# vwxyzjn/cleanrl

Measured on NVIDIA H100. Metric: env steps/sec (SPS) PPO Breakout num_envs=1024, higher is better.
Workload: dtype bf16

## Files before the change

### cleanrl_b200/csrc/net_tc.cu

```cuda
#include <cuda.h>
#include <algorithm>
#include "tc_base.cuh"
#include "tc_conv_win.cuh"
#include "tc_conv23.cuh"
#include "tc_conv1_u8.cuh"
#include "tc_gemm_tma.cuh"
#include "tc_wgrad_win.cuh"
#include "tc_reduce.cuh"
#include "tc_aux.cuh"
#include "tc_heads.cuh"
#include "tc_heads_wide.cuh"
#include "tc_lstm.cuh"

namespace b200rl {

struct NatureLayout {
    int A;
    int64_t c1w, c1b, c2w, c2b, c3w, c3b, fcw, fcb, hw, hb, total;
    int64_t w1f, w2f, w2dg, w3f, w3dg, wfcf, wfcdg, w1l, w1sc, packed_total;
    bool wide; int G; int64_t whf, whdg, hbp;
    int64_t wih, whh, bih, bhh, whhp;
    explicit NatureLayout(int A_) : A(A_), wih(-1), whh(-1), bih(-1), bhh(-1), whhp(-1) {
        int64_t o = 0;
        c1w = o; o += 32 * 4 * 8 * 8;  c1b = o; o += 32;
// ... 406 lines not shown
                   "naturecnn_backward: bad obs_format %d", obs_format);
    B200RL_REQUIRE(obs_format != B200RL_OBS_S2D_U8 || (obs_aux && aligned(obs_aux, 16)), "naturecnn_backward: the uint8 rollout needs obs_aux");
    const NatureLayout L(A);
    const NatureActs Q(n, obs_format == B200RL_OBS_U8_NCHW);
    const bf16* P = reinterpret_cast<const bf16*>(packed);
    bf16* act = reinterpret_cast<bf16*>(acts);
    cudaStream_t s = (cudaStream_t)stream;
    const bf16* x0 = obs_format == B200RL_OBS_U8_NCHW ? act + Q.x0 : reinterpret_cast<const bf16*>(obs);
    const int64_t* x0rows = obs_format == B200RL_OBS_U8_NCHW ? nullptr : rows;
    const size_t big = (naturecnn_big_bytes(n, L) + 255) & ~(size_t)255;
    float* wsbig = reinterpret_cast<float*>(workspace);
    float* wssmall = reinterpret_cast<float*>(reinterpret_cast<char*>(workspace) + big);
    int rc;
    const int A1 = A + 1;
    if (L.wide) {
        ProfScope ps(s, "heads_bwd", 4.0 * n * 512 * A1, (double)n * (2048 + 64 + 8 * A1));
        if ((rc = wide_head_bwd(L, P, dhead, n, A1, act + Q.hid, act + Q.dhid, reinterpret_cast<const uint32_t*>(act + Q.m4),
                                grads + L.hw, grads + L.hb, wsbig, wssmall, s))) return rc;
    } else
    {
        ProfScope ps(s, "heads_bwd", 4.0 * n * 512 * A1, (double)n * (2048 + 64 + 8 * A1));
        if ((rc = heads_bwd_weight<512>(dhead, act + Q.hid, n, A1, wssmall, grads + L.hw, grads + L.hb, s, "naturecnn/heads_bwd"))) return rc;
        if ((rc = heads_bwd_data<512>(dhead, params + L.hw, reinterpret_cast<const uint8_t*>(act + Q.m4), n, A1, act + Q.dhid, s,
                                      "naturecnn/heads_bwd"))) return rc;
    }
    if ((rc = trunk_bwd(L, Q, P, act, grads, n, wsbig, wssmall, tail_ready_event, obs_format == B200RL_OBS_S2D_U8, s))) return rc;
    const bool u8 = obs_format == B200RL_OBS_S2D_U8;
    const WPlan pl = conv1_wgrad_plan(n, u8);
    if (u8) {
        Conv21BwdU8Params cw;
        memset(&cw, 0, sizeof(cw));
        cw.rows = rows; cw.n = (int)n; cw.rows_per_cta = pl.rows_per_cta; cw.ws = wsbig; cw.wsb = wssmall;
        cw.w2dg = P + L.w2dg; cw.m1 = reinterpret_cast<const uint32_t*>(act + Q.m1);
        { ProfScope ps(s, "conv21_bwd", 2.0 * 2.0 * n * 400 * 32 * 256, (double)n * (7744 * 2 + 1600 + 28224 + 14112 * 2));
          if ((rc = launch_conv21_bwd_u8(cw, obs, rows ? (int64_t)1 << 24 : n, act + Q.dact2b, act + Q.dact1, pl.splits, s,
                                         "naturecnn/conv21_bwd_u8"))) return rc; }
    } else {
        WGradWinParams gw;
        wgw_defaults(gw);
        gw.X = x0; gw.rows = x0rows; gw.M = n * 512; gw.n = (int)n; gw.G = 441; gw.cpr = 1; gw.nslots = 4; gw.WRX = round8(128 + 22);
        gw.tpi_shift = 2; gw.n_images = x0rows ? (int64_t)1 << 24 : n;
        gw.shift[0] = 0; gw.shift[1] = 1; gw.shift[2] = 21; gw.shift[3] = 22;
        for (int k = 0; k < 4; ++k) { gw.slot_tap[k] = k; gw.slot_cc[k] = 0; }
        gw.Y = act + Q.dact1; gw.ldy = 32; gw.ncolsY = 32;
        gw.rows_per_cta = pl.rows_per_cta; gw.ws = wsbig; gw.wsb = wssmall;
        { ProfScope ps(s, "conv1_wgrad", 2.0 * n * 400 * 32 * 256, (double)n * (28224 + 14112) * 2);
          if ((rc = launch_wgrad_win(gw, pl.splits, s, "naturecnn/conv1_wgrad"))) return rc; }
    }
    FoldWin fw;
    memset(&fw, 0, sizeof(fw));
    fw.layer = 1; fw.S = pl.splits; fw.nslots = 4; fw.Cout = 32;
    fw.scale = u8 ? 1.0f / 255.0f / kDact1Scale : 1.0f / 255.0f;
    fw.bscale = u8 ? 1.0f / kDact1Scale : 1.f;
    for (int k = 0; k < 4; ++k) fw.slot_tap[k] = k;
    { ProfScope ps(s, "wgrad_fold_bias", 0, 0);
      fw.wsb = wssmall; fw.db = grads + L.c1b;
      tc_fold_win<<<(unsigned)ceil_div(256 * 32 + 32, 32), 256, 0, s>>>(wsbig, fw, grads + L.c1w);
      if ((rc = check_launch("naturecnn/conv1_fold"))) return rc; }
    return B200RL_OK;
}

namespace b200rl {
constexpr int64_t kLstmMaxRows = (int64_t)1 << 17;

struct LstmActs {
    NatureActs T;
    int64_t gx, hseq, hm, save, cm, dgates, total;
    explicit LstmActs(int64_t M) : T(M, false) {
// ... 194 lines not shown
```

### cleanrl_b200/csrc/tc_base.cuh

```cuda
#pragma once
#include <cuda.h>
#include <cstring>
#include "common.cuh"
#include "tc_common.cuh"

namespace b200rl {
using namespace tc;
typedef __nv_bfloat16 bf16;

__device__ __forceinline__ int4 ldg16(const void* p) { return __ldg(reinterpret_cast<const int4*>(p)); }

typedef CUresult (*EncodeTiledFn)(CUtensorMap*, CUtensorMapDataType, cuuint32_t, void*, const cuuint64_t*, const cuuint64_t*,
                                  const cuuint32_t*, const cuuint32_t*, CUtensorMapInterleave, CUtensorMapSwizzle,
                                  CUtensorMapL2promotion, CUtensorMapFloatOOBfill);
static EncodeTiledFn g_encode = nullptr;
static int make_tmap_2d(CUtensorMap* tm, const void* base, int64_t rows, int64_t cols, int box_rows, const char* what) {
    if (!g_encode) {
        void* fn = nullptr;
        cudaDriverEntryPointQueryResult qres;
        cudaError_t e = cudaGetDriverEntryPoint("cuTensorMapEncodeTiled", &fn, cudaEnableDefault, &qres);
        if (e != cudaSuccess || qres != cudaDriverEntryPointSuccess || !fn)
            return fail(B200RL_ERR_CUDA, "%s: cuTensorMapEncodeTiled not available (%s)", what, cudaGetErrorString(e));
        g_encode = reinterpret_cast<EncodeTiledFn>(fn);
    }
    const cuuint64_t dims[2] = {(cuuint64_t)cols, (cuuint64_t)rows};
    const cuuint64_t strides[1] = {(cuuint64_t)cols * 2};
    const cuuint32_t box[2] = {64u, (cuuint32_t)box_rows};
    const cuuint32_t estr[2] = {1u, 1u};
    CUresult r = g_encode(tm, CU_TENSOR_MAP_DATA_TYPE_BFLOAT16, 2, const_cast<void*>(base), dims, strides, box, estr,
                          CU_TENSOR_MAP_INTERLEAVE_NONE, CU_TENSOR_MAP_SWIZZLE_128B, CU_TENSOR_MAP_L2_PROMOTION_L2_256B,
                          CU_TENSOR_MAP_FLOAT_OOB_FILL_NONE);
    if (r != CUDA_SUCCESS) return fail(B200RL_ERR_CUDA, "%s: cuTensorMapEncodeTiled failed (%d)", what, (int)r);
    return B200RL_OK;
}

static int make_tmap_3d(CUtensorMap* tm, const void* base, int64_t n_images, int64_t rows_per_image, int64_t cols, int box_rows,
                        const char* what) {
    if (!g_encode) {
        CUtensorMap dummy;
        int rc = make_tmap_2d(&dummy, base, 128, 64, 8, what);
        if (rc) return rc;
    }
    const cuuint64_t dims[3] = {(cuuint64_t)cols, (cuuint64_t)rows_per_image, (cuuint64_t)n_images};
    const cuuint64_t strides[2] = {(cuuint64_t)cols * 2, (cuuint64_t)rows_per_image * (cuuint64_t)cols * 2};
    const cuuint32_t box[3] = {64u, (cuuint32_t)box_rows, 1u};
    const cuuint32_t estr[3] = {1u, 1u, 1u};
    CUresult r = g_encode(tm, CU_TENSOR_MAP_DATA_TYPE_BFLOAT16, 3, const_cast<void*>(base), dims, strides, box, estr,
                          CU_TENSOR_MAP_INTERLEAVE_NONE, CU_TENSOR_MAP_SWIZZLE_128B, CU_TENSOR_MAP_L2_PROMOTION_L2_256B,
                          CU_TENSOR_MAP_FLOAT_OOB_FILL_NONE);
    if (r != CUDA_SUCCESS) return fail(B200RL_ERR_CUDA, "%s: cuTensorMapEncodeTiled (3-D) failed (%d)", what, (int)r);
    return B200RL_OK;
}

static int make_tmap_3d_u8(CUtensorMap* tm, const void* base, int64_t n_images, int64_t rows_per_image, int64_t cols, int64_t pitch,
                           int box_rows, int box_cols, const char* what) {
    if (!g_encode) {
        CUtensorMap dummy;
        int rc = make_tmap_2d(&dummy, base, 128, 64, 8, what);
        if (rc) return rc;
    }
    const cuuint64_t dims[3] = {(cuuint64_t)cols, (cuuint64_t)rows_per_image, (cuuint64_t)n_images};
    const cuuint64_t strides[2] = {(cuuint64_t)pitch, (cuuint64_t)rows_per_image * (cuuint64_t)pitch};
    const cuuint32_t box[3] = {(cuuint32_t)box_cols, (cuuint32_t)box_rows, 1u};
    const cuuint32_t estr[3] = {1u, 1u, 1u};
    CUresult r = g_encode(tm, CU_TENSOR_MAP_DATA_TYPE_UINT8, 3, const_cast<void*>(base), dims, strides, box, estr,
                          CU_TENSOR_MAP_INTERLEAVE_NONE,
                          box_cols == 64 ? CU_TENSOR_MAP_SWIZZLE_64B : (box_cols == 128 ? CU_TENSOR_MAP_SWIZZLE_128B : CU_TENSOR_MAP_SWIZZLE_NONE),
                          CU_TENSOR_MAP_L2_PROMOTION_L2_256B, CU_TENSOR_MAP_FLOAT_OOB_FILL_NONE);
    if (r != CUDA_SUCCESS) return fail(B200RL_ERR_CUDA, "%s: cuTensorMapEncodeTiled (u8 3-D) failed (%d)", what, (int)r);
    return B200RL_OK;
}

static int make_tmap_pairs_u8(CUtensorMap* tm, const void* base, int64_t n_images, int box_rows, bool swizzle, const char* what) {
    if (!g_encode) {
        CUtensorMap dummy;
        int rc = make_tmap_2d(&dummy, base, 128, 64, 8, what);
        if (rc) return rc;
    }
    const cuuint64_t dims[3] = {128u, 221u, (cuuint64_t)n_images};
    const cuuint64_t strides[2] = {128u, 28224u};
    const cuuint32_t box[3] = {128u, (cuuint32_t)box_rows, 1u};
    const cuuint32_t estr[3] = {1u, 1u, 1u};
    CUresult r = g_encode(tm, CU_TENSOR_MAP_DATA_TYPE_UINT8, 3, const_cast<void*>(base), dims, strides, box, estr,
// ... 33 lines not shown
```

### cleanrl_b200/csrc/tc_common.cuh

```cuda
#pragma once
#include <cuda_bf16.h>
#include <cstdint>
#include "tc_wgmma.cuh"

namespace b200rl { namespace tc {

__device__ __forceinline__ uint32_t smem_u32(const void* p) {
    return static_cast<uint32_t>(__cvta_generic_to_shared(p));
}

__device__ __forceinline__ void mbar_init(uint64_t* bar, uint32_t count) {
    asm volatile("mbarrier.init.shared::cta.b64 [%0], %1;" ::"r"(smem_u32(bar)), "r"(count) : "memory");
}
__device__ __forceinline__ void fence_barrier_init() {
    asm volatile("fence.mbarrier_init.release.cluster;" ::: "memory");
}
__device__ __forceinline__ bool mbar_try_wait(uint64_t* bar, uint32_t parity) {
    uint32_t ok;
    asm volatile(
        "{\n\t.reg .pred p;\n\t"
        "mbarrier.try_wait.parity.shared::cta.b64 p, [%1], %2;\n\t"
        "selp.u32 %0, 1, 0, p;\n\t}\n"
        : "=r"(ok)
        : "r"(smem_u32(bar)), "r"(parity)
        : "memory");
    return ok != 0;
}
#ifndef B200RL_WAIT_MODE
#define B200RL_WAIT_MODE 0
#endif
__device__ __forceinline__ bool mbar_try_wait_hint(uint64_t* bar, uint32_t parity, uint32_t ns) {
    uint32_t ok;
    asm volatile(
        "{\n\t.reg .pred p;\n\t"
        "mbarrier.try_wait.parity.shared::cta.b64 p, [%1], %2, %3;\n\t"
        "selp.u32 %0, 1, 0, p;\n\t}\n"
        : "=r"(ok)
        : "r"(smem_u32(bar)), "r"(parity), "r"(ns)
        : "memory");
    return ok != 0;
}
__device__ __forceinline__ void mbar_wait(uint64_t* bar, uint32_t parity) {
    if (mbar_try_wait(bar, parity)) return;
    const long long t0 = clock64();
#if B200RL_WAIT_MODE == 1
    while (!mbar_try_wait_hint(bar, parity, 1000000u)) {
#elif B200RL_WAIT_MODE == 2
    while (!mbar_try_wait(bar, parity)) {
        __nanosleep(40);
#else
    while (!mbar_try_wait(bar, parity)) {
#endif
        if (clock64() - t0 > (1ll << 33)) __trap();
    }
}

__device__ __forceinline__ void mbar_wait2(uint64_t* bar_a, uint32_t parity_a, uint64_t* bar_b, uint32_t parity_b) {
    const bool a = mbar_try_wait(bar_a, parity_a), b = mbar_try_wait(bar_b, parity_b);
    if (a && b) return;
    if (!a) mbar_wait(bar_a, parity_a);
    if (!b) mbar_wait(bar_b, parity_b);
}

__device__ __forceinline__ void st_global_32b(void* p, const int4& a, const int4& b) {
    reinterpret_cast<int4*>(p)[0] = a;
    reinterpret_cast<int4*>(p)[1] = b;
}

__device__ __forceinline__ void fence_proxy_async_smem() {
    asm volatile("fence.proxy.async.shared::cta;" ::: "memory");
}

constexpr uint64_t kDescSwizzle128 = 1ull << 62;
constexpr uint64_t kDescSwizzle64 = 2ull << 62;

__device__ __forceinline__ uint64_t desc_kmajor(uint32_t smem_addr) {
    return (uint64_t)((smem_addr & 0x3FFFFu) >> 4) | (1ull << 16) | (64ull << 32) | kDescSwizzle128;
}
__device__ __forceinline__ uint64_t desc_mnmajor(uint32_t smem_addr, uint32_t lbo_bytes) {
    return (uint64_t)((smem_addr & 0x3FFFFu) >> 4) | ((uint64_t)((lbo_bytes >> 4) & 0x3FFF) << 16) | (64ull << 32) |
           kDescSwizzle128;
}

template <int R>
__device__ __forceinline__ void stage_acc(float* st, int ld, int wg_tid, const float (&d)[R]) {
    const int row = ((wg_tid >> 5) << 4) + ((wg_tid & 31) >> 2), col = (wg_tid & 3) * 2;
#pragma unroll
// ... 54 lines not shown
```

### cleanrl_b200/csrc/tc_conv1_u8.cuh

```cuda
#pragma once
#include "tc_base.cuh"
#include <cuda_fp16.h>
#include "tc_conv_win.cuh"

namespace b200rl {
using namespace tc;

__device__ __forceinline__ uint64_t desc_kmajor_sw64(uint32_t smem_addr) {
    return (uint64_t)((smem_addr & 0x3FFFFu) >> 4) | (1ull << 16) | (32ull << 32) | kDescSwizzle64;
}
__device__ __forceinline__ uint64_t desc_mnmajor_sw64(uint32_t smem_addr, uint32_t lbo) {
    return (uint64_t)((smem_addr & 0x3FFFFu) >> 4) | ((uint64_t)((lbo >> 4) & 0x3FFF) << 16) | (32ull << 32) | kDescSwizzle64;
}
__device__ __forceinline__ uint32_t img64_off(int r, int c) { return (uint32_t)(r * 64 + ((c ^ ((r >> 1) & 3)) << 4)); }
constexpr int kS2dThreads = 256;
__global__ void __launch_bounds__(kS2dThreads) tc_frames_to_s2d_u8(const uint8_t* __restrict__ obs, const int64_t* __restrict__ rows,
                                                                   int64_t n, uint8_t* __restrict__ out_rm, uint8_t* __restrict__ out_cm) {
    __shared__ __align__(16) uint8_t frame[28224];
    const int64_t i = blockIdx.x;
    const int64_t img = rows ? rows[i] : i;
    const int4* src = reinterpret_cast<const int4*>(obs + img * 28224);
#pragma unroll
    for (int k = 0; k < 7; ++k) {
        const int t = threadIdx.x + k * kS2dThreads;
        if (t < 1764) reinterpret_cast<int4*>(frame)[t] = __ldg(src + t);
    }
    __syncthreads();
    int4* rm = reinterpret_cast<int4*>(out_rm + i * 441 * 64);
    for (int t = threadIdx.x; t < 441 * 4; t += kS2dThreads) {
        const int pos = t >> 2, c = t & 3;
        const int Y = (pos * 3121) >> 16, X = pos - Y * 21;
        const uint8_t* p = frame + c * 7056 + (Y * 4) * 84 + X * 4;
        int4 v;
        v.x = *reinterpret_cast<const int*>(p); v.y = *reinterpret_cast<const int*>(p + 84);
        v.z = *reinterpret_cast<const int*>(p + 168); v.w = *reinterpret_cast<const int*>(p + 252);
// ... 163 lines not shown
                        const float f1 = fmaf((float)(acc[e][4 * j + 2 * hr + 1] * 128 + acc[e][4 * (j + 4) + 2 * hr + 1]), s_sc[co + 1],
                                              s_bias[co + 1]);
                        bits |= (f0 > 0.f ? 1u : 0u) << co;
                        bits |= (f1 > 0.f ? 1u : 0u) << (co + 1);
                        pk[j] = pack_bf16x2_relu(f0, f1);
                    }
                    bits |= __shfl_xor_sync(0xffffffffu, bits, 1);
                    bits |= __shfl_xor_sync(0xffffffffu, bits, 2);
                    if (valid) {
                        if (qd == 0) p.mask_out[cell * 4 + cls] = bits;
                        uint32_t* dst = reinterpret_cast<uint32_t*>(reinterpret_cast<uint8_t*>(p.out) + (cell * 4 + cls) * 64);
#pragma unroll
                        for (int j = 0; j < 4; ++j) dst[4 * j + qd] = pk[j];
                    }
                }
            }
        }
    }
}

struct Conv21BwdU8Params {
    const int64_t* rows;
    int n;
    int64_t rows_per_cta;
    const bf16* w2dg;
    const uint32_t* m1;
    float* ws;
    float* wsb;
};
constexpr int kC1WXStages = 4, kC21WinStages = 2;
constexpr int kC1WXRows = 33, kC1WXBytes = kC1WXRows * 128, kC1WF16Bytes = 136 * 128;
constexpr int kC1WYBytes = 128 * 64, kC1WYPadRows = 24, kC1WYPad = kC1WYPadRows * 64;
constexpr int kC1WShift = 21;
constexpr int kC21WinRows = 140, kC21WinBytes = 18 * 1024;
constexpr int kC21W2Bytes = 4 * 128 * 128;
constexpr int kC21ImgBytes = kC1WYPad + 4 * kC1WYBytes;
constexpr int kC21MaskBytes = 100 * 16;
constexpr size_t kC21Smem = (size_t)kC21W2Bytes + (size_t)kC21WinStages * (kC21WinBytes + kC21MaskBytes) + 2 * (size_t)kC21ImgBytes +
                            2 * (size_t)kC1WF16Bytes + (size_t)kC1WXStages * kC1WXBytes + 1024;
static_assert(kC21Smem + 4608 <= 227 * 1024, "conv21_bwd: shared memory exceeds 227 KB");
static_assert((kC21W2Bytes + kC21WinStages * kC21WinBytes + 2 * kC21ImgBytes) % 1024 == 0, "the fp16 images need 1 KB alignment");
constexpr float kDact1Scale = 4096.0f;

__device__ __forceinline__ uint32_t prmt(uint32_t a, uint32_t b, uint32_t sel) {
    uint32_t d;
    asm("prmt.b32 %0, %1, %2, %3;" : "=r"(d) : "r"(a), "r"(b), "r"(sel));
    return d;
}
constexpr float kU8Bias = 1024.0f;
__device__ __forceinline__ void u8x16_to_f16_biased(const uint4& v, uint4& lo, uint4& hi) {
    constexpr uint32_t k64 = 0x64646464u;
    lo = make_uint4(prmt(v.x, k64, 0x5140u), prmt(v.x, k64, 0x7362u), prmt(v.y, k64, 0x5140u), prmt(v.y, k64, 0x7362u));
    hi = make_uint4(prmt(v.z, k64, 0x5140u), prmt(v.z, k64, 0x7362u), prmt(v.w, k64, 0x5140u), prmt(v.w, k64, 0x7362u));
}
__device__ __forceinline__ uint4 lds128(uint32_t addr) {
    uint4 v;
    asm volatile("ld.shared.v4.u32 {%0, %1, %2, %3}, [%4];" : "=r"(v.x), "=r"(v.y), "=r"(v.z), "=r"(v.w) : "r"(addr) : "memory");
    return v;
}
__device__ __forceinline__ void sts128(uint32_t addr, const uint4& v) {
    asm volatile("st.shared.v4.u32 [%0], {%1, %2, %3, %4};" ::"r"(addr), "r"(v.x), "r"(v.y), "r"(v.z), "r"(v.w) : "memory");
}
__device__ __forceinline__ uint32_t pack_f16x2_sat(float lo, float hi) {
    uint32_t d;
    asm("cvt.rn.satfinite.f16x2.f32 %0, %1, %2;" : "=r"(d) : "f"(hi), "f"(lo));
    return d;
}

__device__ __forceinline__ void sts32(uint32_t addr, uint32_t v) { asm volatile("st.shared.u32 [%0], %1;" ::"r"(addr), "r"(v) : "memory"); }
__device__ __forceinline__ void tma_store_3d(const void* tmap, uint32_t smem_src, int x, int y, int z) {
    asm volatile("cp.async.bulk.tensor.3d.global.shared::cta.bulk_group [%0, {%1, %2, %3}], [%4];"
                 ::"l"(reinterpret_cast<uint64_t>(tmap)), "r"(x), "r"(y), "r"(z), "r"(smem_src) : "memory");
}
__device__ __forceinline__ void bulk_commit() { asm volatile("cp.async.bulk.commit_group;" ::: "memory"); }
template <int N> __device__ __forceinline__ void bulk_wait_read() { asm volatile("cp.async.bulk.wait_group.read %0;" ::"n"(N) : "memory"); }
template <int N> __device__ __forceinline__ void bulk_wait() { asm volatile("cp.async.bulk.wait_group %0;" ::"n"(N) : "memory"); }
__device__ __forceinline__ void bulk_load(uint32_t smem_dst, const void* src, uint32_t bytes, uint64_t* bar) {
    asm volatile("cp.async.bulk.shared::cluster.global.mbarrier::complete_tx::bytes [%0], [%1], %2, [%3];"
                 ::"r"(smem_dst), "l"(src), "r"(bytes), "r"(smem_u32(bar)) : "memory");
}

constexpr int kC1WThreads = 512;
__global__ void __launch_bounds__(kC1WThreads, 1) tc_conv21_bwd_u8(const __grid_constant__ CUtensorMap tmX, const __grid_constant__ CUtensorMap tmWin,
                                                                 const __grid_constant__ CUtensorMap tmY, const Conv21BwdU8Params p) {
    constexpr int XS = kC1WXStages, WS = kC21WinStages;
    extern __shared__ uint8_t smem_raw[];
    __shared__ uint64_t xfull[XS], xempty[XS], wfull[WS], wempty[WS], yfull[2], yempty[2], ffull[2], fempty[2];
    __shared__ float sRed[32 * 32], sBias[32];
    uint8_t* smem = reinterpret_cast<uint8_t*>((reinterpret_cast<uintptr_t>(smem_raw) + 1023) & ~uintptr_t(1023));
    uint8_t* sW2 = smem;
    uint8_t* sWin = sW2 + kC21W2Bytes;
    uint8_t* sImg = sWin + (size_t)WS * kC21WinBytes;
    uint8_t* sF = sImg + 2 * (size_t)kC21ImgBytes;
    uint8_t* sX = sF + 2 * (size_t)kC1WF16Bytes;
    uint8_t* sM = sX + (size_t)XS * kC1WXBytes;
    const int tid = threadIdx.x, warp = tid >> 5, lane = tid & 31;
    if (tid == 0) {
        for (int s = 0; s < XS; ++s) { mbar_init(&xfull[s], 1); mbar_init(&xempty[s], 4); }
        for (int s = 0; s < WS; ++s) { mbar_init(&wfull[s], 1); mbar_init(&wempty[s], 4); }
        for (int s = 0; s < 2; ++s) {
            mbar_init(&yfull[s], 1); mbar_init(&yempty[s], 4);
            mbar_init(&ffull[s], 4); mbar_init(&fempty[s], 4);
        }
        fence_barrier_init();
        tma_prefetch_desc(&tmX);
        tma_prefetch_desc(&tmWin);
        tma_prefetch_desc(&tmY);
    }
    for (int idx = tid; idx < 4 * 128 * 8; idx += blockDim.x) {
        const int c16 = idx & 7, r = (idx >> 3) & 127, t = idx >> 10;
        *reinterpret_cast<int4*>(sW2 + t * (128 * 128) + img_off(r, c16)) = ldg16(p.w2dg + r * 256 + t * 64 + c16 * 8);
    }
    for (int idx = tid; idx < 2 * kC21ImgBytes / 16; idx += blockDim.x) reinterpret_cast<int4*>(sImg)[idx] = make_int4(0, 0, 0, 0);
    fence_proxy_async_smem();
    __syncthreads();
    const int64_t M = (int64_t)p.n * 512;
    const int64_t m_begin = (int64_t)blockIdx.x * p.rows_per_cta;
    int64_t m_end = m_begin + p.rows_per_cta;
    if (m_end > M) m_end = M;
    const int nsteps = (int)((m_end - m_begin) >> 7);
    const int nimg = nsteps >> 2;
    const int img0 = (int)(m_begin >> 9);

    if (warp < 4) {
        if (warp == 0 && lane == 0) {
            auto image_of = [&](int j) -> int { return p.rows ? (int)__ldg(p.rows + img0 + j) : img0 + j; };
            int z = 0, z_next = image_of(0);
            for (int k = 0; k < nsteps; ++k) {
                if ((k & 3) == 0) {
                    z = z_next;
                    if ((k >> 2) + 1 < nimg) z_next = image_of((k >> 2) + 1);
                }
#pragma unroll
                for (int hb = 0; hb < 2; ++hb) {
                    const int j = 2 * k + hb, xs = j % XS;
                    if (j >= XS) mbar_wait(&xempty[xs], ((j / XS) - 1) & 1);
                    mbar_arrive_expect_tx(&xfull[xs], (uint32_t)kC1WXBytes);
                    tma_load_3d(smem_u32(sX + (size_t)xs * kC1WXBytes), &tmX, 0, (k & 3) * 64 + hb * 32, z, &xfull[xs]);
                }
            }
        } else if (warp == 1 && lane == 0) {
            for (int j = 0; j < nimg; ++j) {
                const int s = j % WS;
                if (j >= WS) mbar_wait(&wempty[s], ((j / WS) - 1) & 1);
                mbar_arrive_expect_tx(&wfull[s], (uint32_t)(kC21WinRows * 128 + kC21MaskBytes));
                tma_load_2d(smem_u32(sWin + (size_t)s * kC21WinBytes), &tmWin, 0, (img0 + j) * 121, &wfull[s]);
                bulk_load(smem_u32(sM + (size_t)s * kC21MaskBytes), p.m1 + (int64_t)(img0 + j) * 100 * 4, (uint32_t)kC21MaskBytes, &wfull[s]);
            }
        }
    } else if (warp < 8) {
        const int wt = tid - 128, lane4 = lane >> 2, qd = lane & 3;
        const uint32_t w_base = smem_u32(sW2);
        const int rq = wt >> 2, c16 = wt & 3;
        float bsum[8];
#pragma unroll
        for (int e = 0; e < 8; ++e) bsum[e] = 0.f;
        for (int j = 0; j < nimg; ++j) {
            const int i = img0 + j, buf = j & 1, s = j % WS;
            const uint32_t img = smem_u32(sImg + (size_t)buf * kC21ImgBytes) + kC1WYPad;
            const uint32_t masks = smem_u32(sM + (size_t)s * kC21MaskBytes);
            mbar_wait(&wfull[s], (j / WS) & 1);
            if (j >= 2) mbar_wait(&yempty[buf], ((j >> 1) - 1) & 1);
            if (wt == 0) bulk_wait_read<1>();
            named_bar(1, 128);
#pragma unroll 1
            for (int h2 = 0; h2 < 2; ++h2) {
                float d[64];
                wgmma_fence();
                const uint32_t win = smem_u32(sWin + (size_t)s * kC21WinBytes) + (uint32_t)(h2 * 64 * 128);
                constexpr int shift[4] = {12, 11, 1, 0};
#pragma unroll
                for (int t = 0; t < 4; ++t) {
                    const uint64_t a = desc_kmajor(win + (uint32_t)shift[t] * 128u);
                    const uint64_t b = desc_kmajor(w_base + (uint32_t)(t * 128 * 128));
#pragma unroll
                    for (int kk = 0; kk < 4; ++kk) WgmmaBf16<128, 0, 0>::mma(d, a + 2 * kk, b + 2 * kk, (t | kk) != 0 ? 1u : 0u);
                }
                wgmma_commit();
                int pos[2];
                uint4 mb[2];
#pragma unroll
                for (int hr = 0; hr < 2; ++hr) {
                    const int r = h2 * 64 + ((wt >> 5) << 4) + lane4 + 8 * hr;
                    const int Y = (r * 5958) >> 16, X = r - Y * 11;
                    const bool valid = Y < 10 && X < 10;
                    pos[hr] = valid ? 2 * Y * 21 + 2 * X : -1;
                    mb[hr] = make_uint4(0u, 0u, 0u, 0u);
                    if (valid) mb[hr] = lds128(masks + (uint32_t)(Y * 10 + X) * 16u);
                }
                wgmma_wait<0>();
                wgmma_fence_operands(d);
#pragma unroll
                for (int hr = 0; hr < 2; ++hr) {
                    if (pos[hr] < 0) continue;
                    const uint32_t mw[4] = {mb[hr].x, mb[hr].y, mb[hr].z, mb[hr].w};
#pragma unroll
                    for (int jj = 0; jj < 16; ++jj) {
                        const int g = jj >> 2, c = 8 * (jj & 3) + 2 * qd;
                        float f0 = d[4 * jj + 2 * hr] * kDact1Scale, f1 = d[4 * jj + 2 * hr + 1] * kDact1Scale;
                        if (!((mw[g] >> c) & 1u)) f0 = 0.f;
                        if (!((mw[g] >> (c + 1)) & 1u)) f1 = 0.f;
                        const int q = pos[hr] + (g >> 1) * 21 + (g & 1);
                        sts32(img + img64_off(q, c >> 3) + (uint32_t)((c & 7) * 2), pack_f16x2_sat(f0, f1));
                    }
                }
                __syncwarp();
                if (h2 == 1 && lane == 0) mbar_arrive(&wempty[s]);
            }
            fence_proxy_async_smem();
            named_bar(1, 128);
            if (wt == 0) {
                mbar_arrive(&yfull[buf]);
#pragma unroll
                for (int k = 0; k < 4; ++k) tma_store_3d(&tmY, img + (uint32_t)(k * kC1WYBytes), 0, k * 128, i);
                bulk_commit();
            }
#pragma unroll 1
            for (int st = 0; st < 4; ++st) {
#pragma unroll
                for (int ps = 0; ps < 4; ++ps) {
                    const uint4 v = lds128(img + (uint32_t)(st * kC1WYBytes) + img64_off(ps * 32 + rq, c16));
                    const uint32_t w[4] = {v.x, v.y, v.z, v.w};
#pragma unroll
                    for (int e = 0; e < 4; ++e) {
                        const float2 f = __half22float2(*reinterpret_cast<const __half2*>(&w[e]));
                        bsum[2 * e] += f.x;
                        bsum[2 * e + 1] += f.y;
                    }
                }
            }
        }
        if (wt == 0) bulk_wait<0>();
#pragma unroll
        for (int e = 0; e < 8; ++e) sRed[rq * 32 + c16 * 8 + e] = bsum[e];
        named_bar(1, 128);
        if (wt < 32) {
            float t = 0.f;
#pragma unroll
            for (int l = 0; l < 32; ++l) t += sRed[l * 32 + wt];
            p.wsb[(int64_t)blockIdx.x * 64 + wt] = t;
            sBias[wt] = t * kU8Bias;
        }
        named_bar(2, 256);
    } else if (warp < 12) {
        const int wt = tid & 127, qd = lane & 3;
        float d[64];
#pragma unroll
        for (int e = 0; e < 64; ++e) d[e] = 0.f;
        auto step = [&](int it) {
            const int fs = it & 1, buf = (it >> 2) & 1;
            if ((it & 3) == 0) mbar_wait(&yfull[buf], (it >> 3) & 1);
            mbar_wait(&ffull[fs], (it >> 1) & 1);
            wgmma_fence();
            const uint32_t ystep = smem_u32(sImg + (size_t)buf * kC21ImgBytes) + (uint32_t)(kC1WYPad + (it & 3) * kC1WYBytes);
            const uint64_t ad = desc_mnmajor_sw64(ystep - kC1WShift * 64, kC1WShift * 64);
            const uint64_t bd = desc_mnmajor(smem_u32(sF + (size_t)fs * kC1WF16Bytes), 128);
#pragma unroll
            for (int kk = 0; kk < 8; ++kk) WgmmaF16N128<1, 1>::mma(d, ad + 64 * kk, bd + 128 * kk, (it | kk) != 0 ? 1u : 0u);
            wgmma_commit();
        };
        for (int it = 0; it + 1 < nsteps; ++it) {
            step(it);
            wgmma_wait<1>();
            if (it > 0 && lane == 0) {
                mbar_arrive(&fempty[(it - 1) & 1]);
                if (((it - 1) & 3) == 3) mbar_arrive(&yempty[((it - 1) >> 2) & 1]);
            }
        }
        step(nsteps - 1);
        wgmma_wait<0>();
        wgmma_fence_operands(d);
        named_bar(2, 256);
        const int m = ((wt >> 5) << 4) + (lane >> 2), b = m < 32 ? 1 : 0, co = m & 31;
        const float bias0 = sBias[co], bias8 = sBias[co + 8];
        float* wsc = p.ws + (int64_t)blockIdx.x * 256 * 64;
#pragma unroll
        for (int j = 0; j < 16; ++j) {
            const int h = j >> 3, c = 8 * (j & 7) + 2 * qd;
            float* q = wsc + (int64_t)((2 * b + h) * 64 + c) * 64 + co;
            q[0] = d[4 * j] - bias0;
            q[64] = d[4 * j + 1] - bias0;
            q[8] = d[4 * j + 2] - bias8;
            q[64 + 8] = d[4 * j + 3] - bias8;
        }
    } else {
        const int wt = tid & 127;
        for (int it = 0; it < nsteps; ++it) {
            const int fs = it & 1;
            const uint32_t img = smem_u32(sF + (size_t)fs * kC1WF16Bytes);
            if (it >= 2) mbar_wait(&fempty[fs], ((it >> 1) - 1) & 1);
#pragma unroll
            for (int hb = 0; hb < 2; ++hb) {
                const int j = 2 * it + hb, xs = j % XS;
                const uint32_t blk = smem_u32(sX + (size_t)xs * kC1WXBytes);
                const int nch = (64 + hb) * 4;
                mbar_wait(&xfull[xs], (j / XS) & 1);
                uint4 v[3];
#pragma unroll
                for (int i = 0; i < 2 + hb; ++i)
                    if (wt + 128 * i < nch) v[i] = lds128(blk + (uint32_t)(wt + 128 * i) * 16u);
#pragma unroll
                for (int i = 0; i < 2 + hb; ++i) {
                    const int t = wt + 128 * i;
                    if (t < nch) {
                        const int r = 64 * hb + (t >> 2), c = t & 3;
                        uint4 lo, hi;
                        u8x16_to_f16_biased(v[i], lo, hi);
                        sts128(img + (uint32_t)(r * 128 + (((2 * c) ^ (r & 7)) << 4)), lo);
                        sts128(img + (uint32_t)(r * 128 + (((2 * c + 1) ^ (r & 7)) << 4)), hi);
                    }
                }
                __syncwarp();
                if (lane == 0) mbar_arrive(&xempty[xs]);
            }
            fence_proxy_async_smem();
            __syncwarp();
            if (lane == 0) mbar_arrive(&ffull[fs]);
        }
    }
}

static int launch_conv21_bwd_u8(const Conv21BwdU8Params& p, const void* frames_rm, int64_t n_images, const bf16* dact2b, void* dact1_f16,
                                int ctas, cudaStream_t s, const char* what) {
    int rc;
    if (p.rows_per_cta % 512 != 0) return fail(B200RL_ERR_INVALID_ARGUMENT, "%s: a CTA must own whole images (512 grid rows)", what);
    if (ctas < 1 || (int64_t)(ctas - 1) * p.rows_per_cta >= (int64_t)p.n * 512)
        return fail(B200RL_ERR_INVALID_ARGUMENT, "%s: every CTA must own at least one image", what);
    CUtensorMap tmX, tmWin, tmY;
    memset(&tmX, 0, sizeof(tmX)); memset(&tmWin, 0, sizeof(tmWin)); memset(&tmY, 0, sizeof(tmY));
    if ((rc = make_tmap_pairs_u8(&tmX, frames_rm, n_images, kC1WXRows, false, what))) return rc;
    if ((rc = make_tmap_2d(&tmWin, dact2b, (int64_t)p.n * 121, 64, kC21WinRows, what))) return rc;
    if ((rc = make_tmap_3d_u8(&tmY, dact1_f16, p.n, 441, 64, 64, 128, 64, what))) return rc;
    static SmemAttrCache attr;
    if ((rc = attr.ensure(tc_conv21_bwd_u8, kC21Smem, what))) return rc;
    tc_conv21_bwd_u8<<<ctas, kC1WThreads, kC21Smem, s>>>(tmX, tmWin, tmY, p);
    return check_launch(what);
}

constexpr int kConv1I8Stages = 8;
static int launch_conv1_i8(const Conv1U8Params& p, const void* frames_rm, cudaStream_t s, const char* what) {
    constexpr int STAGES = kConv1I8Stages;
    const size_t smem = (size_t)4 * 64 * 64 + (size_t)STAGES * 144 * 128 + 1024;
    const int total = p.n * 2;
    int grid = num_sms();
    if (grid > total) grid = total;
    CUtensorMap tmA, tmW;
    memset(&tmA, 0, sizeof(tmA));
    memset(&tmW, 0, sizeof(tmW));
    int rc = make_tmap_pairs_u8(&tmA, frames_rm, p.n_images, 144, true, what);
    if (rc) return rc;
    if ((rc = make_tmap_3d_u8(&tmW, p.limbs, 1, 64, 256, 256, 64, 64, what))) return rc;
    static SmemAttrCache attr;
    if ((rc = attr.ensure(tc_conv1_i8<STAGES>, smem, what))) return rc;
    tc_conv1_i8<STAGES><<<grid, kConv1I8Threads, smem, s>>>(tmA, tmW, p, total);
    return check_launch(what);
}

}
```

### cleanrl_b200/csrc/tc_wgmma.cuh

```cuda
#pragma once
#include <cstdint>

namespace b200rl { namespace tc {

__device__ __forceinline__ void wgmma_fence() { asm volatile("wgmma.fence.sync.aligned;" ::: "memory"); }
__device__ __forceinline__ void wgmma_commit() { asm volatile("wgmma.commit_group.sync.aligned;" ::: "memory"); }
template <int N>
__device__ __forceinline__ void wgmma_wait() { asm volatile("wgmma.wait_group.sync.aligned %0;" ::"n"(N) : "memory"); }
template <class T, int R>
__device__ __forceinline__ void wgmma_fence_operands(T (&d)[R]) {
#pragma unroll
    for (int i = 0; i < R; ++i) asm volatile("" : "+r"(reinterpret_cast<uint32_t&>(d[i]))::"memory");
}

template <int N, int TA, int TB> struct WgmmaBf16;
template <int TA, int TB> struct WgmmaBf16<32, TA, TB> {
    __device__ __forceinline__ static void mma(float (&d)[16], uint64_t adesc, uint64_t bdesc, uint32_t accumulate) {
        asm volatile(
            "{\n\t.reg .pred p;\n\tsetp.ne.b32 p, %18, 0;\n\t"
            "wgmma.mma_async.sync.aligned.m64n32k16.f32.bf16.bf16 {"
            "%0, %1, %2, %3, %4, %5, %6, %7, %8, %9, %10, %11, %12, %13, %14, %15"
            "}, %16, %17, p, 1, 1, %19, %20;\n\t}\n"
            : "+f"(d[0]), "+f"(d[1]), "+f"(d[2]), "+f"(d[3]), "+f"(d[4]), "+f"(d[5]), "+f"(d[6]), "+f"(d[7]),
              "+f"(d[8]), "+f"(d[9]), "+f"(d[10]), "+f"(d[11]), "+f"(d[12]), "+f"(d[13]), "+f"(d[14]), "+f"(d[15])
            : "l"(adesc), "l"(bdesc), "r"(accumulate), "n"(TA), "n"(TB));
    }
};
template <int TA, int TB> struct WgmmaBf16<64, TA, TB> {
    __device__ __forceinline__ static void mma(float (&d)[32], uint64_t adesc, uint64_t bdesc, uint32_t accumulate) {
        asm volatile(
            "{\n\t.reg .pred p;\n\tsetp.ne.b32 p, %34, 0;\n\t"
            "wgmma.mma_async.sync.aligned.m64n64k16.f32.bf16.bf16 {"
            "%0, %1, %2, %3, %4, %5, %6, %7, %8, %9, %10, %11, %12, %13, %14, %15, "
            "%16, %17, %18, %19, %20, %21, %22, %23, %24, %25, %26, %27, %28, %29, %30, %31"
            "}, %32, %33, p, 1, 1, %35, %36;\n\t}\n"
            : "+f"(d[0]), "+f"(d[1]), "+f"(d[2]), "+f"(d[3]), "+f"(d[4]), "+f"(d[5]), "+f"(d[6]), "+f"(d[7]),
              "+f"(d[8]), "+f"(d[9]), "+f"(d[10]), "+f"(d[11]), "+f"(d[12]), "+f"(d[13]), "+f"(d[14]), "+f"(d[15]),
              "+f"(d[16]), "+f"(d[17]), "+f"(d[18]), "+f"(d[19]), "+f"(d[20]), "+f"(d[21]), "+f"(d[22]), "+f"(d[23]),
              "+f"(d[24]), "+f"(d[25]), "+f"(d[26]), "+f"(d[27]), "+f"(d[28]), "+f"(d[29]), "+f"(d[30]), "+f"(d[31])
            : "l"(adesc), "l"(bdesc), "r"(accumulate), "n"(TA), "n"(TB));
    }
};
template <int TA, int TB> struct WgmmaBf16<96, TA, TB> {
    __device__ __forceinline__ static void mma(float (&d)[48], uint64_t adesc, uint64_t bdesc, uint32_t accumulate) {
        asm volatile(
// ... 135 lines not shown
```

Before: 1.421 million.

## Pipeline conv21 backward wgmma across images and read unpadded dact2 via 4-D TMA

Restructures the dgrad warpgroup of the fused conv2/conv1 backward kernel to double-buffer accumulators, so the next half-image's wgmma is issued while the current epilogue masks and stores. Register budgets are redistributed with setmaxnreg between producer, dgrad and expand warpgroups. The d(act2) window is now loaded from the unpadded dact2a tensor through a 4-D TMA map with out-of-bounds zero fill, which removes the dependency on a padded copy. L2 prefetches are added for upcoming frames, windows and masks. Waits now use a bounded wait that traps later, which adds complexity and raises register pressure.

Measured after the change: 1.426 million, median of 6. No clear change (+0.4%).

```diff
diff --git a/cleanrl_b200/csrc/net_tc.cu b/cleanrl_b200/csrc/net_tc.cu
--- a/cleanrl_b200/csrc/net_tc.cu
+++ b/cleanrl_b200/csrc/net_tc.cu
@@ -462,8 +462,8 @@
         memset(&cw, 0, sizeof(cw));
         cw.rows = rows; cw.n = (int)n; cw.rows_per_cta = pl.rows_per_cta; cw.ws = wsbig; cw.wsb = wssmall;
         cw.w2dg = P + L.w2dg; cw.m1 = reinterpret_cast<const uint32_t*>(act + Q.m1);
-        { ProfScope ps(s, "conv21_bwd", 2.0 * 2.0 * n * 400 * 32 * 256, (double)n * (7744 * 2 + 1600 + 28224 + 14112 * 2));
-          if ((rc = launch_conv21_bwd_u8(cw, obs, rows ? (int64_t)1 << 24 : n, act + Q.dact2b, act + Q.dact1, pl.splits, s,
+        { ProfScope ps(s, "conv21_bwd", 2.0 * 2.0 * n * 400 * 32 * 256, (double)n * (5184 * 2 + 1600 + 28224 + 14112 * 2));
+          if ((rc = launch_conv21_bwd_u8(cw, obs, rows ? (int64_t)1 << 24 : n, act + Q.dact2a, act + Q.dact1, pl.splits, s,
                                          "naturecnn/conv21_bwd_u8"))) return rc; }
     } else {
         WGradWinParams gw;
diff --git a/cleanrl_b200/csrc/tc_base.cuh b/cleanrl_b200/csrc/tc_base.cuh
--- a/cleanrl_b200/csrc/tc_base.cuh
+++ b/cleanrl_b200/csrc/tc_base.cuh
@@ -49,6 +49,24 @@
                           CU_TENSOR_MAP_INTERLEAVE_NONE, CU_TENSOR_MAP_SWIZZLE_128B, CU_TENSOR_MAP_L2_PROMOTION_L2_256B,
                           CU_TENSOR_MAP_FLOAT_OOB_FILL_NONE);
     if (r != CUDA_SUCCESS) return fail(B200RL_ERR_CUDA, "%s: cuTensorMapEncodeTiled (3-D) failed (%d)", what, (int)r);
+    return B200RL_OK;
+}
+
+static int make_tmap_grid_4d(CUtensorMap* tm, const void* base, int64_t n_images, int grid, int valid, int box_x, int box_y,
+                             const char* what) {
+    if (!g_encode) {
+        CUtensorMap dummy;
+        int rc = make_tmap_2d(&dummy, base, 128, 64, 8, what);
+        if (rc) return rc;
+    }
+    const cuuint64_t dims[4] = {64u, (cuuint64_t)valid, (cuuint64_t)valid, (cuuint64_t)n_images};
+    const cuuint64_t strides[3] = {128u, (cuuint64_t)grid * 128u, (cuuint64_t)grid * grid * 128u};
+    const cuuint32_t box[4] = {64u, (cuuint32_t)box_x, (cuuint32_t)box_y, 1u};
+    const cuuint32_t estr[4] = {1u, 1u, 1u, 1u};
+    CUresult r = g_encode(tm, CU_TENSOR_MAP_DATA_TYPE_BFLOAT16, 4, const_cast<void*>(base), dims, strides, box, estr,
+                          CU_TENSOR_MAP_INTERLEAVE_NONE, CU_TENSOR_MAP_SWIZZLE_128B, CU_TENSOR_MAP_L2_PROMOTION_L2_256B,
+                          CU_TENSOR_MAP_FLOAT_OOB_FILL_NONE);
+    if (r != CUDA_SUCCESS) return fail(B200RL_ERR_CUDA, "%s: cuTensorMapEncodeTiled (4-D grid) failed (%d)", what, (int)r);
     return B200RL_OK;
 }
 
diff --git a/cleanrl_b200/csrc/tc_common.cuh b/cleanrl_b200/csrc/tc_common.cuh
--- a/cleanrl_b200/csrc/tc_common.cuh
+++ b/cleanrl_b200/csrc/tc_common.cuh
@@ -53,6 +53,14 @@
 #endif
         if (clock64() - t0 > (1ll << 33)) __trap();
     }
+}
+
+__device__ __forceinline__ bool mbar_wait_bounded(uint64_t* bar, uint32_t parity) {
+    if (mbar_try_wait(bar, parity)) return true;
+    const long long t0 = clock64();
+    while (!mbar_try_wait(bar, parity))
+        if (clock64() - t0 > (1ll << 33)) return false;
+    return true;
 }
 
 __device__ __forceinline__ void mbar_wait2(uint64_t* bar_a, uint32_t parity_a, uint64_t* bar_b, uint32_t parity_b) {
diff --git a/cleanrl_b200/csrc/tc_conv1_u8.cuh b/cleanrl_b200/csrc/tc_conv1_u8.cuh
--- a/cleanrl_b200/csrc/tc_conv1_u8.cuh
+++ b/cleanrl_b200/csrc/tc_conv1_u8.cuh
@@ -1,6 +1,7 @@
 #pragma once
 #include "tc_base.cuh"
 #include <cuda_fp16.h>
+#include <type_traits>
 #include "tc_conv_win.cuh"
 
 namespace b200rl {
@@ -230,7 +231,8 @@
 constexpr int kC1WXRows = 33, kC1WXBytes = kC1WXRows * 128, kC1WF16Bytes = 136 * 128;
 constexpr int kC1WYBytes = 128 * 64, kC1WYPadRows = 24, kC1WYPad = kC1WYPadRows * 64;
 constexpr int kC1WShift = 21;
-constexpr int kC21WinRows = 140, kC21WinBytes = 18 * 1024;
+constexpr int kC21WinX = 11, kC21WinY = 13, kC21WinRows = kC21WinX * kC21WinY, kC21WinBytes = 18 * 1024;
+static_assert(kC21WinRows >= 128 + 12 && kC21WinRows * 128 <= kC21WinBytes, "conv21_bwd: the d(act2) window");
 constexpr int kC21W2Bytes = 4 * 128 * 128;
 constexpr int kC21ImgBytes = kC1WYPad + 4 * kC1WYBytes;
 constexpr int kC21MaskBytes = 100 * 16;
@@ -270,6 +272,22 @@
     asm volatile("cp.async.bulk.tensor.3d.global.shared::cta.bulk_group [%0, {%1, %2, %3}], [%4];"
                  ::"l"(reinterpret_cast<uint64_t>(tmap)), "r"(x), "r"(y), "r"(z), "r"(smem_src) : "memory");
 }
+__device__ __forceinline__ void tma_load_4d(uint32_t smem_dst, const void* tmap, int x, int y, int z, int w, uint64_t* bar) {
+    asm volatile("cp.async.bulk.tensor.4d.shared::cluster.global.mbarrier::complete_tx::bytes [%0], [%1, {%2, %3, %4, %5}], [%6];"
+                 ::"r"(smem_dst), "l"(reinterpret_cast<uint64_t>(tmap)), "r"(x), "r"(y), "r"(z), "r"(w), "r"(smem_u32(bar))
+                 : "memory");
+}
+__device__ __forceinline__ void tma_prefetch_3d(const void* tmap, int x, int y, int z) {
+    asm volatile("cp.async.bulk.prefetch.tensor.3d.L2.global.tile [%0, {%1, %2, %3}];"
+                 ::"l"(reinterpret_cast<uint64_t>(tmap)), "r"(x), "r"(y), "r"(z) : "memory");
+}
+__device__ __forceinline__ void tma_prefetch_4d(const void* tmap, int x, int y, int z, int w) {
+    asm volatile("cp.async.bulk.prefetch.tensor.4d.L2.global.tile [%0, {%1, %2, %3, %4}];"
+                 ::"l"(reinterpret_cast<uint64_t>(tmap)), "r"(x), "r"(y), "r"(z), "r"(w) : "memory");
+}
+__device__ __forceinline__ void bulk_prefetch_l2(const void* src, uint32_t bytes) {
+    asm volatile("cp.async.bulk.prefetch.L2.global [%0], %1;" ::"l"(src), "r"(bytes) : "memory");
+}
 __device__ __forceinline__ void bulk_commit() { asm volatile("cp.async.bulk.commit_group;" ::: "memory"); }
 template <int N> __device__ __forceinline__ void bulk_wait_read() { asm volatile("cp.async.bulk.wait_group.read %0;" ::"n"(N) : "memory"); }
 template <int N> __device__ __forceinline__ void bulk_wait() { asm volatile("cp.async.bulk.wait_group %0;" ::"n"(N) : "memory"); }
@@ -279,6 +297,8 @@
 }
 
 constexpr int kC1WThreads = 512;
+constexpr int kC21RegsProducer = 40, kC21RegsDgrad = 240, kC21RegsExpand = 104;
+static_assert(kC21RegsProducer + kC21RegsDgrad + 128 + kC21RegsExpand <= 512, "conv21_bwd: register budgets exceed the SM");
 __global__ void __launch_bounds__(kC1WThreads, 1) tc_conv21_bwd_u8(const __grid_constant__ CUtensorMap tmX, const __grid_constant__ CUtensorMap tmWin,
                                                                  const __grid_constant__ CUtensorMap tmY, const Conv21BwdU8Params p) {
     constexpr int XS = kC1WXStages, WS = kC21WinStages;
@@ -321,6 +341,7 @@
     const int img0 = (int)(m_begin >> 9);
 
     if (warp < 4) {
+        setmaxnreg_dec<kC21RegsProducer>();
         if (warp == 0 && lane == 0) {
             auto image_of = [&](int j) -> int { return p.rows ? (int)__ldg(p.rows + img0 + j) : img0 + j; };
             int z = 0, z_next = image_of(0);
@@ -329,6 +350,10 @@
                     z = z_next;
                     if ((k >> 2) + 1 < nimg) z_next = image_of((k >> 2) + 1);
                 }
+                if ((k >> 2) + 1 < nimg) {
+#pragma unroll
+                    for (int hb = 0; hb < 2; ++hb) tma_prefetch_3d(&tmX, 0, (k & 3) * 64 + hb * 32, z_next);
+                }
 #pragma unroll
                 for (int hb = 0; hb < 2; ++hb) {
                     const int j = 2 * k + hb, xs = j % XS;
@@ -340,71 +365,92 @@
         } else if (warp == 1 && lane == 0) {
             for (int j = 0; j < nimg; ++j) {
                 const int s = j % WS;
+                if (j + WS < nimg) {
+                    tma_prefetch_4d(&tmWin, 0, -1, -1, img0 + j + WS);
+                    bulk_prefetch_l2(p.m1 + (int64_t)(img0 + j + WS) * 100 * 4, (uint32_t)kC21MaskBytes);
+                }
                 if (j >= WS) mbar_wait(&wempty[s], ((j / WS) - 1) & 1);
                 mbar_arrive_expect_tx(&wfull[s], (uint32_t)(kC21WinRows * 128 + kC21MaskBytes));
-                tma_load_2d(smem_u32(sWin + (size_t)s * kC21WinBytes), &tmWin, 0, (img0 + j) * 121, &wfull[s]);
+                tma_load_4d(smem_u32(sWin + (size_t)s * kC21WinBytes), &tmWin, 0, -1, -1, img0 + j, &wfull[s]);
                 bulk_load(smem_u32(sM + (size_t)s * kC21MaskBytes), p.m1 + (int64_t)(img0 + j) * 100 * 4, (uint32_t)kC21MaskBytes, &wfull[s]);
             }
         }
     } else if (warp < 8) {
+        setmaxnreg_inc<kC21RegsDgrad>();
         const int wt = tid - 128, lane4 = lane >> 2, qd = lane & 3;
         const uint32_t w_base = smem_u32(sW2);
         const int rq = wt >> 2, c16 = wt & 3;
         float bsum[8];
 #pragma unroll
         for (int e = 0; e < 8; ++e) bsum[e] = 0.f;
-        for (int j = 0; j < nimg; ++j) {
+        float d0[64], d1[64];
+        bool late = false;
+        auto issue = [&](float (&d)[64], int s, int h2) {
+            wgmma_fence();
+            const uint32_t win = smem_u32(sWin + (size_t)s * kC21WinBytes) + (uint32_t)(h2 * 64 * 128);
+            constexpr int shift[4] = {12, 11, 1, 0};
+#pragma unroll
+            for (int t = 0; t < 4; ++t) {
+                const uint64_t a = desc_kmajor(win + (uint32_t)shift[t] * 128u);
+                const uint64_t b = desc_kmajor(w_base + (uint32_t)(t * 128 * 128));
+#pragma unroll
+                for (int kk = 0; kk < 4; ++kk) WgmmaBf16<128, 0, 0>::mma(d, a + 2 * kk, b + 2 * kk, (t | kk) != 0 ? 1u : 0u);
+            }
+            wgmma_commit();
+        };
+        auto rows_of = [&](int h2, uint32_t masks, int (&pos)[2], uint4 (&mb)[2]) {
+#pragma unroll
+            for (int hr = 0; hr < 2; ++hr) {
+                const int r = h2 * 64 + ((wt >> 5) << 4) + lane4 + 8 * hr;
+                const int Y = (r * 5958) >> 16, X = r - Y * 11;
+                const bool valid = Y < 10 && X < 10;
+                pos[hr] = valid ? 2 * Y * 21 + 2 * X : -1;
+                mb[hr] = make_uint4(0u, 0u, 0u, 0u);
+                if (valid) mb[hr] = lds128(masks + (uint32_t)(Y * 10 + X) * 16u);
+            }
+        };
+        auto epilogue = [&](const float (&d)[64], uint32_t img, const int (&pos)[2], const uint4 (&mb)[2]) {
+#pragma unroll
+            for (int hr = 0; hr < 2; ++hr) {
+                if (pos[hr] < 0) continue;
+                const uint32_t mw[4] = {mb[hr].x, mb[hr].y, mb[hr].z, mb[hr].w};
+#pragma unroll
+                for (int jj = 0; jj < 16; ++jj) {
+                    const int g = jj >> 2, c = 8 * (jj & 3) + 2 * qd;
+                    float f0 = d[4 * jj + 2 * hr] * kDact1Scale, f1 = d[4 * jj + 2 * hr + 1] * kDact1Scale;
+                    if (!((mw[g] >> c) & 1u)) f0 = 0.f;
+                    if (!((mw[g] >> (c + 1)) & 1u)) f1 = 0.f;
+                    const int q = pos[hr] + (g >> 1) * 21 + (g & 1);
+                    sts32(img + img64_off(q, c >> 3) + (uint32_t)((c & 7) * 2), pack_f16x2_sat(f0, f1));
+                }
+            }
+        };
+        auto image = [&](int j, auto more) {
+            constexpr bool kMore = decltype(more)::value;
             const int i = img0 + j, buf = j & 1, s = j % WS;
             const uint32_t img = smem_u32(sImg + (size_t)buf * kC21ImgBytes) + kC1WYPad;
             const uint32_t masks = smem_u32(sM + (size_t)s * kC21MaskBytes);
-            mbar_wait(&wfull[s], (j / WS) & 1);
-            if (j >= 2) mbar_wait(&yempty[buf], ((j >> 1) - 1) & 1);
+            int pos[2];
+            uint4 mb[2];
+            rows_of(0, masks, pos, mb);
+            wgmma_wait<0>();
+            wgmma_fence_operands_f32(d0);
+            issue(d1, s, 1);
+            if (j >= 2 && !late) late = !mbar_wait_bounded(&yempty[buf], ((j >> 1) - 1) & 1);
             if (wt == 0) bulk_wait_read<1>();
             named_bar(1, 128);
-#pragma unroll 1
-            for (int h2 = 0; h2 < 2; ++h2) {
-                float d[64];
-                wgmma_fence();
-                const uint32_t win = smem_u32(sWin + (size_t)s * kC21WinBytes) + (uint32_t)(h2 * 64 * 128);
-                constexpr int shift[4] = {12, 11, 1, 0};
-#pragma unroll
-                for (int t = 0; t < 4; ++t) {
-                    const uint64_t a = desc_kmajor(win + (uint32_t)shift[t] * 128u);
-                    const uint64_t b = desc_kmajor(w_base + (uint32_t)(t * 128 * 128));
-#pragma unroll
-                    for (int kk = 0; kk < 4; ++kk) WgmmaBf16<128, 0, 0>::mma(d, a + 2 * kk, b + 2 * kk, (t | kk) != 0 ? 1u : 0u);
-                }
-                wgmma_commit();
-                int pos[2];
-                uint4 mb[2];
-#pragma unroll
-                for (int hr = 0; hr < 2; ++hr) {
-                    const int r = h2 * 64 + ((wt >> 5) << 4) + lane4 + 8 * hr;
-                    const int Y = (r * 5958) >> 16, X = r - Y * 11;
-                    const bool valid = Y < 10 && X < 10;
-                    pos[hr] = valid ? 2 * Y * 21 + 2 * X : -1;
-                    mb[hr] = make_uint4(0u, 0u, 0u, 0u);
-                    if (valid) mb[hr] = lds128(masks + (uint32_t)(Y * 10 + X) * 16u);
-                }
-                wgmma_wait<0>();
-                wgmma_fence_operands(d);
-#pragma unroll
-                for (int hr = 0; hr < 2; ++hr) {
-                    if (pos[hr] < 0) continue;
-                    const uint32_t mw[4] = {mb[hr].x, mb[hr].y, mb[hr].z, mb[hr].w};
-#pragma unroll
-                    for (int jj = 0; jj < 16; ++jj) {
-                        const int g = jj >> 2, c = 8 * (jj & 3) + 2 * qd;
-                        float f0 = d[4 * jj + 2 * hr] * kDact1Scale, f1 = d[4 * jj + 2 * hr + 1] * kDact1Scale;
-                        if (!((mw[g] >> c) & 1u)) f0 = 0.f;
-                        if (!((mw[g] >> (c + 1)) & 1u)) f1 = 0.f;
-                        const int q = pos[hr] + (g >> 1) * 21 + (g & 1);
-                        sts32(img + img64_off(q, c >> 3) + (uint32_t)((c & 7) * 2), pack_f16x2_sat(f0, f1));
-                    }
-                }
-                __syncwarp();
-                if (h2 == 1 && lane == 0) mbar_arrive(&wempty[s]);
-            }
+            epilogue(d0, img, pos, mb);
+            if constexpr (kMore) {
+                const int sn = (j + 1) % WS;
+                if (!late) late = !mbar_wait_bounded(&wfull[sn], ((j + 1) / WS) & 1);
+                issue(d0, sn, 0);
+            }
+            rows_of(1, masks, pos, mb);
+            if constexpr (kMore) wgmma_wait<1>(); else wgmma_wait<0>();
+            wgmma_fence_operands_f32(d1);
+            epilogue(d1, img, pos, mb);
+            __syncwarp();
+            if (lane == 0) mbar_arrive(&wempty[s]);
             fence_proxy_async_smem();
             named_bar(1, 128);
             if (wt == 0) {
@@ -427,7 +473,12 @@
                     }
                 }
             }
-        }
+        };
+        mbar_wait(&wfull[0], 0);
+        issue(d0, 0, 0);
+        for (int j = 0; j + 1 < nimg; ++j) image(j, std::true_type{});
+        image(nimg - 1, std::false_type{});
+        if (late) __trap();
         if (wt == 0) bulk_wait<0>();
 #pragma unroll
         for (int e = 0; e < 8; ++e) sRed[rq * 32 + c16 * 8 + e] = bsum[e];
@@ -482,6 +533,7 @@
             q[64 + 8] = d[4 * j + 3] - bias8;
         }
     } else {
+        setmaxnreg_dec<kC21RegsExpand>();
         const int wt = tid & 127;
         for (int it = 0; it < nsteps; ++it) {
             const int fs = it & 1;
@@ -518,7 +570,7 @@
     }
 }
 
-static int launch_conv21_bwd_u8(const Conv21BwdU8Params& p, const void* frames_rm, int64_t n_images, const bf16* dact2b, void* dact1_f16,
+static int launch_conv21_bwd_u8(const Conv21BwdU8Params& p, const void* frames_rm, int64_t n_images, const bf16* dact2a, void* dact1_f16,
                                 int ctas, cudaStream_t s, const char* what) {
     int rc;
     if (p.rows_per_cta % 512 != 0) return fail(B200RL_ERR_INVALID_ARGUMENT, "%s: a CTA must own whole images (512 grid rows)", what);
@@ -527,7 +579,7 @@
     CUtensorMap tmX, tmWin, tmY;
     memset(&tmX, 0, sizeof(tmX)); memset(&tmWin, 0, sizeof(tmWin)); memset(&tmY, 0, sizeof(tmY));
     if ((rc = make_tmap_pairs_u8(&tmX, frames_rm, n_images, kC1WXRows, false, what))) return rc;
-    if ((rc = make_tmap_2d(&tmWin, dact2b, (int64_t)p.n * 121, 64, kC21WinRows, what))) return rc;
+    if ((rc = make_tmap_grid_4d(&tmWin, dact2a, p.n, 10, 9, kC21WinX, kC21WinY, what))) return rc;
     if ((rc = make_tmap_3d_u8(&tmY, dact1_f16, p.n, 441, 64, 64, 128, 64, what))) return rc;
     static SmemAttrCache attr;
     if ((rc = attr.ensure(tc_conv21_bwd_u8, kC21Smem, what))) return rc;
diff --git a/cleanrl_b200/csrc/tc_wgmma.cuh b/cleanrl_b200/csrc/tc_wgmma.cuh
--- a/cleanrl_b200/csrc/tc_wgmma.cuh
+++ b/cleanrl_b200/csrc/tc_wgmma.cuh
@@ -11,6 +11,12 @@
 __device__ __forceinline__ void wgmma_fence_operands(T (&d)[R]) {
 #pragma unroll
     for (int i = 0; i < R; ++i) asm volatile("" : "+r"(reinterpret_cast<uint32_t&>(d[i]))::"memory");
+}
+
+template <int R>
+__device__ __forceinline__ void wgmma_fence_operands_f32(float (&d)[R]) {
+#pragma unroll
+    for (int i = 0; i < R; ++i) asm volatile("" : "+f"(d[i])::"memory");
 }
 
 template <int N, int TA, int TB> struct WgmmaBf16;
```
